# yang-song/score_sde_pytorch

Measured on AMD Instinct MI355X. Metric: pc_sampler_images_per_sec, higher is better.
Workload: dtype f32 via 3-way bf16 split, fp32 accumulate (the 1x1 / NIN / Linear GEMMs and the attention forward as exact-fp32 products on the BF16 matrix pipe, fp32 softmax; 3x3 convolutions and the attention backward on the fp32-MFMA kernels)

## Files before the change

### include/ssde.h

```cpp
#ifndef SSDE_H_
#define SSDE_H_

#include <stddef.h>
#include <stdint.h>

#ifdef __cplusplus
extern "C" {
#endif

#define SSDE_ABI_VERSION 10

enum {
  SSDE_PRO_NONE = 0,
  SSDE_PRO_GN = 1,
  SSDE_PRO_GN_SILU = 2,
  SSDE_PRO_SILU = 3
};

typedef struct ssde_src {
  const float* p0;
  const float* p1;
  int32_t c0, c1;
  int32_t pro_mode;
  int32_t gn_groups;
  const float* gn_mean;
  const float* gn_rstd;
  const float* gn_gamma;
  const float* gn_beta;
  uint32_t drop_thresh;
  float drop_scale;
  const uint32_t* drop_seed;
  uint32_t drop_salt;
  int32_t _pad;
} ssde_src;

typedef struct ssde_conv_args {
  ssde_src main;
  ssde_src aux;
  const float* w_main;
  const float* w_aux;
  int32_t n, h_in, w_in;
  int32_t h_out, w_out, c_out;
  int32_t ksize;
  int32_t stride;
  int32_t pad;
  int32_t tile;
  const float* bias;
  const float* chan_add;
  int32_t chan_add_ld;
  int32_t resid_post;
  const float* resid;
  float out_scale;
  uint32_t flags;
  float* dst;
  float* gn_part;
  float* wino_v;
  const float* gn_in_part0;
  const float* gn_in_part1;
  int32_t gn_in_slices0, gn_in_slices1;
  float gn_in_eps;
  int32_t _pad_gn_in;
} ssde_conv_args;

enum { SSDE_CONVF_V_GIVEN = 1u,
       SSDE_CONVF_BF16X6 = 2u,
       SSDE_CONVF_NO_KSPLIT = 4u,
       SSDE_CONVF_BKC8 = 8u,
       SSDE_CONVF_GEMM_PIPE = 16u,
       SSDE_CONVF_NO_GEMM_PIPE = 32u,
       SSDE_CONVF_X6_BM64 = 64u,
       SSDE_CONVF_X6_PF2 = 128u,
       SSDE_CONVF_NO_SMALL_COUT = 256u,
       SSDE_CONVF_X6_WIDE = 512u,
       SSDE_CONVF_X6_NO_WIDE = 1024u };
enum { SSDE_TILE_AUTO = 0, SSDE_TILE_256x64 = 1, SSDE_TILE_128x64 = 2, SSDE_TILE_64x64 = 3, SSDE_TILE_256x32 = 4,
       SSDE_TILE_WINOGRAD = 5,
       SSDE_TILE_WINOGRAD4 = 6,
       SSDE_TILE_WINOGRAD4R = 9 };

typedef struct ssde_gn_stats_args {
  const float* p0; const float* p1; int32_t c0, c1;
  int32_t n, hw, groups; float eps;
  float* mean; float* rstd;
  float* scratch;
  int32_t slices; int32_t _pad0;
} ssde_gn_stats_args;

typedef struct ssde_gn_finalize_args {
  const float* part0; const float* part1;
  int32_t c0, c1, slices0, slices1;
  int32_t n, groups; float eps; int32_t _pad0;
  float* mean; float* rstd;
} ssde_gn_finalize_args;

typedef struct ssde_upfirdn_args {
  ssde_src src;
  int32_t n, h_in, w_in, c;
  int32_t h_out, w_out;
  int32_t up, down, pad0, pad1;
  int32_t kh, kw;
  float k[16];
  float* dst;
  int32_t accumulate;
  int32_t _pad0;
  float* dst2;
} ssde_upfirdn_args;

typedef struct ssde_attn_args {
  const float* qkv; float* dst;
  int32_t n, l, c; float scale;
  uint32_t flags;
  int32_t _pad0;
} ssde_attn_args;
enum { SSDE_ATTNF_BF16X6 = 1u };

typedef struct ssde_embed_args {
  const float* cond;
  const float* w;
  float* dst;
  int32_t n, dim, kind, _pad0;
} ssde_embed_args;

typedef struct ssde_to_nhwc_args {
  const float* src; float* dst; int32_t n, c, h, w, c_pad; float a, b;
  int32_t mode;
  const float* v;
} ssde_to_nhwc_args;
typedef struct ssde_to_nchw_args {
  const float* src; float* dst; int32_t n, c, h, w, c_src;
  int32_t mode;
  const float* v;
  float alpha;
  int32_t accumulate;
} ssde_to_nchw_args;

typedef struct ssde_bias_act_args {
  const float* src; const float* bias; float* dst;
  int64_t numel; int32_t channels; int32_t inner;
  int32_t act;
  float alpha, scale;
  int32_t grad;
  const float* ref;
} ssde_bias_act_args;

typedef struct ssde_sumsq_args {
  const float* a; const float* b; float* out_a; float* out_b; int32_t n, per;
} ssde_sumsq_args;
typedef struct ssde_randn_args {
  float* dst; int64_t numel; uint64_t seed; const int32_t* step_ptr; int32_t stream_id; int32_t _pad0;
  const uint64_t* seed_ptr;
} ssde_randn_args;
typedef struct ssde_langevin_args {
  float* x; float* x_mean; const float* grad; const float* noise;
  const float* grad_sumsq; const float* noise_sumsq;
  const float* alpha_tab; const int32_t* step_ptr;
  int32_t n, per; float snr; int32_t _pad0;
} ssde_langevin_args;
// ... 313 lines not shown
```

### score_sde_pytorch_amd/_lib.py

```python
import ctypes as C
import os

_HERE = os.path.dirname(os.path.abspath(__file__))
LIB_PATH = os.environ.get("SSDE_LIB_PATH") or os.path.join(_HERE, "libssde_hip.so")
ABI_VERSION = 10

PRO_NONE, PRO_GN, PRO_GN_SILU, PRO_SILU = 0, 1, 2, 3
TILE_AUTO, TILE_256x64, TILE_128x64, TILE_64x64, TILE_256x32, TILE_WINOGRAD, TILE_WINOGRAD4 = 0, 1, 2, 3, 4, 5, 6
TILE_WINOGRAD4R = 9
TILES_WINOGRAD4 = (TILE_WINOGRAD4, TILE_WINOGRAD4R)
CONVF_V_GIVEN, CONVF_BF16X6, CONVF_NO_KSPLIT, CONVF_BKC8, CONVF_GEMM_PIPE, CONVF_NO_GEMM_PIPE, CONVF_X6_BM64, CONVF_X6_PF2, \
    CONVF_NO_SMALL_COUT, CONVF_X6_WIDE, CONVF_X6_NO_WIDE = 1, 2, 4, 8, 16, 32, 64, 128, 256, 512, 1024
WGRADF_DIRECT, WGRADF_F2, WGRADF_F4_FORCE, WGRADF_NO_STREAMK, WGRADF_NO_XCD_ORDER, WGRADF_1X1_CHUNKED, WGRADF_XVEC1 = 1, 2, 4, 8, 16, 32, 64
GNBWDF_THREE_KERNELS, GNBWDF_DEFER_PARAMS = 1, 2
(OP_CONV, OP_GN_STATS, OP_UPFIRDN, OP_ATTN, OP_EMBED, OP_TO_NHWC, OP_TO_NCHW, OP_BIAS_ACT, OP_SUMSQ,
 OP_RANDN, OP_LANGEVIN, OP_PREDICTOR, OP_FILL, OP_STEP_INC, OP_WGRAD, OP_COLSUM, OP_GN_BWD_REDUCE, OP_PROLOGUE_BWD,
 OP_ATTN_BWD, OP_PERTURB, OP_DSM_LOSS, OP_SUMSQ_FLAT, OP_ADAM, OP_MEMSET, OP_AXPY, OP_PACK, OP_PROJECT,
 OP_GN_FINALIZE, OP_PF_DRIFT, OP_HUTCH_DIV, OP_COLSUM_FINISH, OP_GN_BWD_FINISH) = range(1, 33)
FINISH_JOBS = 16
COLSUMF_DEFER = 1
PACK_CONV3, PACK_WINO3, PACK_MATRIX, PACK_VECTOR, PACK_WINO4, PACK_WINO4R = 1, 2, 3, 4, 5, 6

_fp = C.c_void_p


class Src(C.Structure):
    _fields_ = [("p0", _fp), ("p1", _fp), ("c0", C.c_int32), ("c1", C.c_int32),
                ("pro_mode", C.c_int32), ("gn_groups", C.c_int32),
                ("gn_mean", _fp), ("gn_rstd", _fp), ("gn_gamma", _fp), ("gn_beta", _fp),
                ("drop_thresh", C.c_uint32), ("drop_scale", C.c_float), ("drop_seed", _fp),
                ("drop_salt", C.c_uint32), ("_pad", C.c_int32)]


class ConvArgs(C.Structure):
    _fields_ = [("main", Src), ("aux", Src), ("w_main", _fp), ("w_aux", _fp),
                ("n", C.c_int32), ("h_in", C.c_int32), ("w_in", C.c_int32),
                ("h_out", C.c_int32), ("w_out", C.c_int32), ("c_out", C.c_int32),
                ("ksize", C.c_int32), ("stride", C.c_int32), ("pad", C.c_int32), ("tile", C.c_int32),
                ("bias", _fp), ("chan_add", _fp), ("chan_add_ld", C.c_int32), ("resid_post", C.c_int32),
                ("resid", _fp), ("out_scale", C.c_float), ("flags", C.c_uint32), ("dst", _fp), ("gn_part", _fp), ("wino_v", _fp),
                ("gn_in_part0", _fp), ("gn_in_part1", _fp), ("gn_in_slices0", C.c_int32), ("gn_in_slices1", C.c_int32),
                ("gn_in_eps", C.c_float), ("_pad_gn_in", C.c_int32)]


class GnStatsArgs(C.Structure):
    _fields_ = [("p0", _fp), ("p1", _fp), ("c0", C.c_int32), ("c1", C.c_int32),
                ("n", C.c_int32), ("hw", C.c_int32), ("groups", C.c_int32), ("eps", C.c_float),
                ("mean", _fp), ("rstd", _fp), ("scratch", _fp), ("slices", C.c_int32), ("_pad0", C.c_int32)]


class RkCombineArgs(C.Structure):
    _fields_ = [("y", _fp), ("k", _fp), ("n", C.c_int64), ("terms", C.c_int32), ("_pad0", C.c_int32), ("coef", C.c_double * 7),
                ("dst", _fp), ("dst32", _fp), ("n32", C.c_int64)]


class RkErrorArgs(C.Structure):
    _fields_ = [("y", _fp), ("y_new", _fp), ("k", _fp), ("n", C.c_int64), ("coef", C.c_double * 7), ("atol", C.c_double),
                ("rtol", C.c_double), ("partial", _fp), ("partial_len", C.c_int32), ("_pad0", C.c_int32), ("out", _fp)]


class PfDriftArgs(C.Structure):
    _fields_ = [("x", _fp), ("score", _fp), ("dst", _fp), ("numel", C.c_int64), ("a", C.c_float), ("g2", C.c_float), ("dyn", _fp)]


class OdeDyn(C.Structure):
    _fields_ = [("label", C.c_float), ("std", C.c_float), ("a", C.c_float), ("g2", C.c_float), ("dst", _fp)]


class HutchDivArgs(C.Structure):
    _fields_ = [("gx", _fp), ("eps", _fp), ("dst", _fp), ("dst_off", C.c_int64), ("n", C.c_int32), ("per", C.c_int32),
                ("a", C.c_float), ("g2", C.c_float), ("dyn", _fp)]


class GnFinalizeArgs(C.Structure):
    _fields_ = [("part0", _fp), ("part1", _fp), ("c0", C.c_int32), ("c1", C.c_int32), ("slices0", C.c_int32), ("slices1", C.c_int32),
                ("n", C.c_int32), ("groups", C.c_int32), ("eps", C.c_float), ("_pad0", C.c_int32), ("mean", _fp), ("rstd", _fp)]


class UpfirdnArgs(C.Structure):
    _fields_ = [("src", Src), ("n", C.c_int32), ("h_in", C.c_int32), ("w_in", C.c_int32), ("c", C.c_int32),
                ("h_out", C.c_int32), ("w_out", C.c_int32),
                ("up", C.c_int32), ("down", C.c_int32), ("pad0", C.c_int32), ("pad1", C.c_int32),
                ("kh", C.c_int32), ("kw", C.c_int32), ("k", C.c_float * 16), ("dst", _fp),
                ("accumulate", C.c_int32), ("_pad0", C.c_int32), ("dst2", _fp)]


class AttnArgs(C.Structure):
    _fields_ = [("qkv", _fp), ("dst", _fp), ("n", C.c_int32), ("l", C.c_int32), ("c", C.c_int32), ("scale", C.c_float),
                ("flags", C.c_uint32), ("_pad0", C.c_int32)]


class EmbedArgs(C.Structure):
    _fields_ = [("cond", _fp), ("w", _fp), ("dst", _fp), ("n", C.c_int32), ("dim", C.c_int32),
                ("kind", C.c_int32), ("_pad0", C.c_int32)]

# ... 120 lines not shown


class MemsetArgs(C.Structure):
    _fields_ = [("dst", _fp), ("bytes", C.c_int64), ("value", C.c_int32), ("_pad0", C.c_int32)]


class AxpyArgs(C.Structure):
    _fields_ = [("x", _fp), ("gate", _fp), ("dst", _fp), ("numel", C.c_int64), ("alpha", C.c_float), ("acc", C.c_int32)]


class PackDesc(C.Structure):
    _fields_ = [("src", _fp), ("src2", _fp), ("dst", _fp), ("kind", C.c_int32), ("cout", C.c_int32), ("cin", C.c_int32),
                ("cout_l", C.c_int32), ("cin_l", C.c_int32), ("flags", C.c_int32), ("r_off", C.c_int32), ("c_off", C.c_int32),
                ("n", C.c_int64)]


class PackArgs(C.Structure):
    _fields_ = [("table", _fp), ("count", C.c_int32), ("kind", C.c_int32), ("max_n", C.c_int64)]


class _OpUnion(C.Union):
    _fields_ = [("conv", ConvArgs), ("gn", GnStatsArgs), ("fir", UpfirdnArgs), ("attn", AttnArgs),
                ("embed", EmbedArgs), ("to_nhwc", ToNhwcArgs), ("to_nchw", ToNchwArgs), ("bias_act", BiasActArgs),
                ("sumsq", SumsqArgs), ("randn", RandnArgs), ("langevin", LangevinArgs), ("predictor", PredictorArgs),
                ("fill", FillArgs), ("step_inc", StepIncArgs),
                ("wgrad", WgradArgs), ("colsum", ColsumArgs), ("gn_bwd", GnBwdReduceArgs), ("pro_bwd", PrologueBwdArgs),
                ("attn_bwd", AttnBwdArgs), ("perturb", PerturbArgs), ("dsm_loss", DsmLossArgs),
                ("sumsq_flat", SumsqFlatArgs), ("adam", AdamArgs), ("memset", MemsetArgs), ("axpy", AxpyArgs),
                ("pack", PackArgs), ("project", ProjectArgs), ("gn_fin", GnFinalizeArgs),
                ("pf_drift", PfDriftArgs), ("hutch_div", HutchDivArgs), ("colsum_fin", ColsumFinishArgs), ("gn_bwd_fin", GnBwdFinishArgs)]


class Op(C.Structure):
    _fields_ = [("kind", C.c_int32), ("flops_class", C.c_int32), ("u", _OpUnion)]


_UNION_FIELD = {OP_CONV: "conv", OP_GN_STATS: "gn", OP_UPFIRDN: "fir", OP_ATTN: "attn", OP_EMBED: "embed",
                OP_TO_NHWC: "to_nhwc", OP_TO_NCHW: "to_nchw", OP_BIAS_ACT: "bias_act", OP_SUMSQ: "sumsq",
                OP_RANDN: "randn", OP_LANGEVIN: "langevin", OP_PREDICTOR: "predictor", OP_FILL: "fill",
                OP_STEP_INC: "step_inc", OP_WGRAD: "wgrad", OP_COLSUM: "colsum", OP_GN_BWD_REDUCE: "gn_bwd",
                OP_PROLOGUE_BWD: "pro_bwd", OP_ATTN_BWD: "attn_bwd", OP_PERTURB: "perturb", OP_DSM_LOSS: "dsm_loss",
                OP_SUMSQ_FLAT: "sumsq_flat", OP_ADAM: "adam", OP_MEMSET: "memset", OP_AXPY: "axpy", OP_PACK: "pack", OP_PROJECT: "project",
                OP_GN_FINALIZE: "gn_fin", OP_PF_DRIFT: "pf_drift", OP_HUTCH_DIV: "hutch_div", OP_COLSUM_FINISH: "colsum_fin",
                OP_GN_BWD_FINISH: "gn_bwd_fin"}

EXPORTS = ["ssde_conv2d", "ssde_groupnorm_stats", "ssde_upfirdn2d", "ssde_attention", "ssde_embed", "ssde_to_nhwc",
           "ssde_to_nchw", "ssde_fused_bias_act", "ssde_sumsq", "ssde_randn", "ssde_langevin_update",
           "ssde_predictor_update", "ssde_fill_from_table", "ssde_step_inc", "ssde_program_run",
           "ssde_program_run_timed", "ssde_graph_capture", "ssde_graph_launch", "ssde_graph_destroy",
           "ssde_abi_version", "ssde_sizeof_op", "ssde_last_error", "ssde_conv_lds_bytes",
           "ssde_conv_wgrad", "ssde_colsum", "ssde_gn_bwd_reduce", "ssde_prologue_bwd", "ssde_attention_bwd",
           "ssde_perturb", "ssde_dsm_loss", "ssde_sumsq_flat", "ssde_adam_clip_ema", "ssde_memset", "ssde_axpy",
           "ssde_wgrad_scratch_floats", "ssde_wgrad_wants_winograd4", "ssde_pack_weights", "ssde_project_update", "ssde_gn_finalize", "ssde_conv_gn_slices", "ssde_rk_combine", "ssde_rk_error_norm", "ssde_pf_drift", "ssde_hutch_div", "ssde_sample_update", "ssde_mfma_probe", "ssde_colsum_finish", "ssde_gn_bwd_finish", "ssde_gn_bwd_scratch_rows",
           "ssde_plan_load", "ssde_plan_load_file", "ssde_plan_destroy", "ssde_plan_info", "ssde_plan_param",
           "ssde_plan_refresh_weights", "ssde_unet_forward", "ssde_pc_reset", "ssde_pc_run", "ssde_pc_state",
           "ssde_train_step", "ssde_train_forward", "ssde_unet_backward", "ssde_plan_copy_io"]

_lib = None


def conv_route_flags(env=None):
    e = os.environ if env is None else env
    f = 0
    if e.get("SSDE_MATRIX", "").startswith("b"):
        f |= CONVF_BF16X6
    if e.get("SSDE_CONV_KSPLIT", "1") == "0":
        f |= CONVF_NO_KSPLIT
    if e.get("SSDE_CONV_BKC64", "") == "8":
        f |= CONVF_BKC8
    if e.get("SSDE_GEMM_PIPE", "") == "0":
        f |= CONVF_NO_GEMM_PIPE
    if e.get("SSDE_GEMM_PIPE", "") == "2":
        f |= CONVF_GEMM_PIPE
    if e.get("SSDE_X6_BM", "") == "64":
        f |= CONVF_X6_BM64
    if e.get("SSDE_X6_PF", "") == "2":
        f |= CONVF_X6_PF2
    if e.get("SSDE_CONV_SMALL", "1") == "0":
        f |= CONVF_NO_SMALL_COUT
    if e.get("SSDE_X6_WIDE", "") == "1":
        f |= CONVF_X6_WIDE
    if e.get("SSDE_X6_WIDE", "") == "0":
        f |= CONVF_X6_NO_WIDE
    return f


ATTNF_BF16X6 = 1


def attn_route_flags(env=None):
    e = os.environ if env is None else env
    return ATTNF_BF16X6 if e.get("SSDE_MATRIX", "").startswith("b") and e.get("SSDE_ATTN_X6", "1") != "0" else 0


def wgrad_route_flags(env=None):
    e = os.environ if env is None else env
    f = {"0": WGRADF_DIRECT, "2": WGRADF_F2, "44": WGRADF_F4_FORCE}.get(e.get("SSDE_WGRAD_WINOGRAD", ""), 0)
    if e.get("SSDE_WGRAD4_STREAMK", "1") == "0":
        f |= WGRADF_NO_STREAMK
    if e.get("SSDE_WGRAD4_XCD", "1") == "0":
        f |= WGRADF_NO_XCD_ORDER
    if e.get("SSDE_WGRAD_1X1_PIPELINED", "1") == "0":
        f |= WGRADF_1X1_CHUNKED
    if e.get("SSDE_WGRAD4_XVEC", "2") == "1":
        f |= WGRADF_XVEC1
    return f


def gn_bwd_route_flags(env=None):
    e = os.environ if env is None else env
    return GNBWDF_THREE_KERNELS if e.get("SSDE_GN_BWD_FUSED", "1") == "0" else 0


class SsdeError(RuntimeError):
    pass


def bind(lib):
    for name in EXPORTS:
        if not hasattr(lib, name):
            raise SsdeError("libssde_hip.so does not export %s" % name)
    lib.ssde_last_error.restype = C.c_char_p
    lib.ssde_program_run.argtypes = [C.POINTER(Op), C.c_int32, C.c_void_p]
    lib.ssde_program_run_timed.argtypes = [C.POINTER(Op), C.c_int32, C.c_void_p, C.POINTER(C.c_float)]
    lib.ssde_graph_capture.argtypes = [C.POINTER(Op), C.c_int32, C.c_void_p, C.POINTER(C.c_void_p)]
    lib.ssde_graph_launch.argtypes = [C.c_void_p, C.c_void_p]
    lib.ssde_graph_destroy.argtypes = [C.c_void_p]
    for name, typ in [("ssde_conv2d", ConvArgs), ("ssde_groupnorm_stats", GnStatsArgs), ("ssde_upfirdn2d", UpfirdnArgs),
                      ("ssde_attention", AttnArgs), ("ssde_embed", EmbedArgs), ("ssde_to_nhwc", ToNhwcArgs),
                      ("ssde_to_nchw", ToNchwArgs), ("ssde_fused_bias_act", BiasActArgs), ("ssde_sumsq", SumsqArgs),
                      ("ssde_randn", RandnArgs), ("ssde_langevin_update", LangevinArgs),
                      ("ssde_predictor_update", PredictorArgs), ("ssde_fill_from_table", FillArgs),
                      ("ssde_step_inc", StepIncArgs), ("ssde_conv_wgrad", WgradArgs), ("ssde_colsum", ColsumArgs),
                      ("ssde_gn_bwd_reduce", GnBwdReduceArgs), ("ssde_prologue_bwd", PrologueBwdArgs),
                      ("ssde_attention_bwd", AttnBwdArgs), ("ssde_perturb", PerturbArgs), ("ssde_dsm_loss", DsmLossArgs),
                      ("ssde_sumsq_flat", SumsqFlatArgs), ("ssde_adam_clip_ema", AdamArgs), ("ssde_memset", MemsetArgs),
                      ("ssde_axpy", AxpyArgs), ("ssde_pack_weights", PackArgs), ("ssde_project_update", ProjectArgs),
                      ("ssde_gn_finalize", GnFinalizeArgs), ("ssde_rk_combine", RkCombineArgs), ("ssde_hutch_div", HutchDivArgs), ("ssde_sample_update", SampleUpdateArgs),
                      ("ssde_rk_error_norm", RkErrorArgs), ("ssde_pf_drift", PfDriftArgs),
                      ("ssde_colsum_finish", ColsumFinishArgs), ("ssde_gn_bwd_finish", GnBwdFinishArgs)]:
        getattr(lib, name).argtypes = [C.POINTER(typ), C.c_void_p]
    lib.ssde_conv_lds_bytes.argtypes = [C.POINTER(ConvArgs)]
    lib.ssde_conv_gn_slices.argtypes = [C.POINTER(ConvArgs)]
    lib.ssde_wgrad_scratch_floats.argtypes = [C.POINTER(WgradArgs)]
    lib.ssde_wgrad_scratch_floats.restype = C.c_int64
    lib.ssde_wgrad_wants_winograd4.argtypes = [C.POINTER(WgradArgs)]
    lib.ssde_gn_bwd_scratch_rows.argtypes = [C.POINTER(GnBwdReduceArgs)]
    if lib.ssde_abi_version() != ABI_VERSION:
        raise SsdeError("ABI mismatch: library %d, binding %d" % (lib.ssde_abi_version(), ABI_VERSION))
    if lib.ssde_sizeof_op() != C.sizeof(Op):
        raise SsdeError("struct layout mismatch: sizeof(ssde_op) library %d, ctypes %d" % (lib.ssde_sizeof_op(), C.sizeof(Op)))
    return lib


def load():
    global _lib
    if _lib is not None:
        return _lib
    if not os.path.exists(LIB_PATH):
        raise SsdeError(
            "libssde_hip.so not found at %s -- build it with `python -c 'import __graft_entry__ as g; g.build()'` "
            "(score_sde_pytorch_amd has no CPU/eager fallback)" % LIB_PATH)
    lib = bind(C.CDLL(LIB_PATH))
    _lib = lib
    return lib

# ... 35 lines not shown
```

### score_sde_pytorch_amd/csrc/conv_mfma.hip

```cpp
#include "ssde_common.h"

typedef float f32x16 __attribute__((ext_vector_type(16)));

namespace {

struct ConvGeom {
  int N, Hin, Win, Hout, Wout, Cout, CoutPad;
  int stride, pad;
  int lTW, lTH;
  int tiles_x, tiles_per_img;
  int m_tiles, n_tiles;
};

struct ConvKParams {
  ssde_src main, aux;
  const float* w_main;
  const float* w_aux;
  ConvGeom g;
  const float* bias;
  const float* chan_add;
  int chan_add_ld;
  const float* resid;
  int resid_post;
  float scale;
// ... 107 lines not shown
        const int r = (q >> 1) / BN;
        const int tap = r % T, cb = r / T;
        const int cin8 = ch * NB8 + cb;
        if (cin8 < ncin8)
          bv[it] = *reinterpret_cast<const float4*>(
              wpk + ((size_t)(cin8 * T + tap) * g.CoutPad + n0 + j) * 8 + f * 4);
      }
    }
#pragma unroll
    for (int it = 0; it < MAXI; ++it) { mu[it] = 0.f; rs[it] = 1.f; }
    if (pro.gn && (c_base + f4 * 4) < Ctot) {
      gam = *reinterpret_cast<const float4*>(s.gn_gamma + c_base + f4 * 4);
      bet = *reinterpret_cast<const float4*>(s.gn_beta + c_base + f4 * 4);
      const int gidx = (c_base + f4 * 4) / cpg;
#pragma unroll
      for (int it = 0; it < MAXI; ++it)
        if (goff[it] >= 0) {
          mu[it] = s.gn_mean[gimg[it] * s.gn_groups + gidx];
          rs[it] = s.gn_rstd[gimg[it] * s.gn_groups + gidx];
        }
    }
  };
  auto store_stage = [&]() {
#pragma unroll
    for (int it = 0; it < MAXI; ++it) {
      if (goff[it] == -2) continue;
      float4 v = av[it];
      if (goff[it] >= 0 && chan_ok)
        v = ssde_pro_apply(v, mu[it], rs[it], gam, bet, (uint32_t)goff[it] * (uint32_t)Ctot + (uint32_t)(c_stage + f4 * 4), pro);
      const int q = tid + it * kThreads;
      *reinterpret_cast<float4*>(As + (q / F4) * LDA + f4 * 4) = v;
    }
#pragma unroll
    for (int it = 0; it < B_ITERS; ++it) {
      const int q = tid + it * kThreads;
      if (B_ITEMS % kThreads == 0 || q < B_ITEMS) {
        const int f = q & 1;
        const int j = (q >> 1) % BN;
        const int r = (q >> 1) / BN;
        const int tap = r % T, cb = r / T;
        *reinterpret_cast<float4*>(Bs + (tap * BN + j) * LDA + cb * 8 + f * 4) = bv[it];
      }
    }
  };

  if (ch0 >= ch1) return;
  load_stage(ch0);
  __syncthreads();
  store_stage();
  __syncthreads();
  for (int ch = ch0; ch < ch1; ++ch) {
    const bool has_next = ch + 1 < ch1;
    if (has_next) load_stage(ch + 1);
#pragma unroll
    for (int tap = 0; tap < T; ++tap) {
      const int dy = tap / KS, dx = tap % KS;
      const int aoff = (dy * HWd + dx) * LDA;
#pragma unroll
      for (int kk = 0; kk < NB8; ++kk) {
        float4 af[TM], bf[TN];
#pragma unroll
        for (int a = 0; a < TM; ++a) af[a] = *reinterpret_cast<const float4*>(As + hb[a] + aoff + kk * 8);
#pragma unroll
        for (int b = 0; b < TN; ++b) bf[b] = *reinterpret_cast<const float4*>(Bs + bb[b] + tap * BN * LDA + kk * 8);
#pragma unroll
        for (int a = 0; a < TM; ++a)
#pragma unroll
          for (int b = 0; b < TN; ++b) {
            acc[a][b] = __builtin_amdgcn_mfma_f32_32x32x2f32(af[a].x, bf[b].x, acc[a][b], 0, 0, 0);
            acc[a][b] = __builtin_amdgcn_mfma_f32_32x32x2f32(af[a].y, bf[b].y, acc[a][b], 0, 0, 0);
            acc[a][b] = __builtin_amdgcn_mfma_f32_32x32x2f32(af[a].z, bf[b].z, acc[a][b], 0, 0, 0);
            acc[a][b] = __builtin_amdgcn_mfma_f32_32x32x2f32(af[a].w, bf[b].w, acc[a][b], 0, 0, 0);
          }
      }
    }
    if (has_next) {
      __syncthreads();
      store_stage();
      __syncthreads();
    }
  }
}

template <int WM, int WN, int TM, int TN, bool HAS3, bool HAS1, int BKC3>
__global__ __launch_bounds__(kThreads, 2) void conv_mfma_kernel(const ConvKParams p) {
  constexpr int BM = WM * TM * 32, BN = WN * TN * 32;
  SSDE_LDS(smem);
  const ConvGeom& g = p.g;

  const int bid = blockIdx.x;
  const int xcd = bid & 7, l = bid >> 3;
  const int nt = l % g.n_tiles;
  const int ks = (l / g.n_tiles) % p.ksplit;
  const int mt = (l / (g.n_tiles * p.ksplit)) * 8 + xcd;
  if (mt >= g.m_tiles) return;

  const int IMGS = BM >> (g.lTW + g.lTH);
  const int img0 = (mt / g.tiles_per_img) * IMGS;
  const int trem = mt % g.tiles_per_img;
  const int ty = trem / g.tiles_x, tx = trem % g.tiles_x;
  const int n0 = nt * BN;

  const int wave = threadIdx.x >> 6;
  const int wm0 = (wave / WN) * (TM * 32);
  const int wn0 = (wave % WN) * (TN * 32);

  f32x16 acc[TM][TN];
#pragma unroll
  for (int a = 0; a < TM; ++a)
#pragma unroll
    for (int b = 0; b < TN; ++b)
#pragma unroll
      for (int r = 0; r < 16; ++r) acc[a][b][r] = 0.f;

  if constexpr (HAS3)
    conv_phase<3, BKC3, BM, BN, TM, TN, 5>(p.main, p.w_main, g, g.stride, g.pad, g.Hin, g.Win,
                                         img0, ty, tx, n0, wm0, wn0, acc, smem, ks, p.ksplit);
  if constexpr (HAS1)
    conv_phase<1, 32, BM, BN, TM, TN, (BM * 8) / kThreads>(p.aux, p.w_aux, g, 1, 0, g.Hout, g.Wout,
                                                          img0, ty, tx, n0, wm0, wn0, acc, smem, ks, p.ksplit);

  const int lane = threadIdx.x & 63;
  const int li = lane & 31, lh = lane >> 5;
  const int TW = 1 << g.lTW, TH = 1 << g.lTH;
  constexpr int LDT = BN + 4;
  __syncthreads();
#pragma unroll
  for (int b = 0; b < TN; ++b)
#pragma unroll
    for (int a = 0; a < TM; ++a)
#pragma unroll
      for (int r = 0; r < 16; ++r) {
        const int m = wm0 + a * 32 + (r & 3) + 8 * (r >> 2) + 4 * lh;
        smem[m * LDT + wn0 + b * 32 + li] = acc[a][b][r];
      }
  __syncthreads();
  auto pixfn = [&](int m, size_t& pix, int& img) {
    const int c = m & (TW - 1);
    const int rr = (m >> g.lTW) & (TH - 1);
    img = img0 + (m >> (g.lTW + g.lTH));
    const int oy = ty * TH + rr, ox = tx * TW + c;
    if (img >= g.N || oy >= g.Hout || ox >= g.Wout) return false;
    pix = ((size_t)img * g.Hout + oy) * g.Wout + ox;
    return true;
  };
  if constexpr (BM == 64 && BN == 64) if (p.ksplit == 2) {
    unsigned* sy = p.sync + 2 * (mt * g.n_tiles + nt);
    int* ticket = reinterpret_cast<int*>(smem + BM * LDT);
    if (threadIdx.x == 0) *ticket = (int)atomicAdd(sy, 1u);
    __syncthreads();
    const bool first = *ticket == 0;
    if (!first) {
      if (threadIdx.x == 0)
        while (__hip_atomic_load(sy + 1, __ATOMIC_RELAXED, __HIP_MEMORY_SCOPE_AGENT) == 0u) __builtin_amdgcn_s_sleep(4);
      __syncthreads();
    }
    constexpr int QN = BN / 4;
    constexpr int ITERS = BM * QN / kThreads;
    float* tp[ITERS];
    float* dp[ITERS];
    float o[ITERS][4];
#pragma unroll
    for (int it = 0; it < ITERS; ++it) {
      const int q = threadIdx.x + it * kThreads;
      const int m = q / QN, j = (q % QN) * 4;
      size_t pix; int img;
      const bool ok = pixfn(m, pix, img) && n0 + j < g.Cout;
      tp[it] = smem + m * LDT + j;
      dp[it] = ok ? p.dst + pix * g.Cout + n0 + j : nullptr;
    }
    if (first) {
#pragma unroll
      for (int it = 0; it < ITERS; ++it)
        if (dp[it]) {
#pragma unroll
          for (int k = 0; k < 4; ++k) __hip_atomic_store(dp[it] + k, tp[it][k], __ATOMIC_RELAXED, __HIP_MEMORY_SCOPE_AGENT);
        }
    } else {
#pragma unroll
      for (int it = 0; it < ITERS; ++it)
#pragma unroll
        for (int k = 0; k < 4; ++k)
          o[it][k] = dp[it] ? __hip_atomic_load(dp[it] + k, __ATOMIC_RELAXED, __HIP_MEMORY_SCOPE_AGENT) : 0.f;
#pragma unroll
      for (int it = 0; it < ITERS; ++it)
#pragma unroll
        for (int k = 0; k < 4; ++k) tp[it][k] += o[it][k];
    }
    if (first) {
      asm volatile("" ::: "memory");
      __builtin_amdgcn_s_waitcnt(0);
      __syncthreads();
      if (threadIdx.x == 0) atomicAdd(sy + 1, 1u);
      return;
    }
    __syncthreads();
    if (threadIdx.x == 0) { sy[0] = 0u; sy[1] = 0u; }
  }
  SsdeEpi e{p.bias, p.chan_add, p.chan_add_ld, p.resid, p.resid_post, p.scale, p.dst, g.Cout, p.gn_part};
  const int gn_entry = p.gn_part ? img0 * g.tiles_per_img + trem : -1;
  const int rpi_log2 = IMGS > 1 ? g.lTW + g.lTH : 30;
  ssde_store_tile<BM, BN, kThreads>(smem, LDT, n0, e, pixfn, gn_entry, rpi_log2, g.N * g.tiles_per_img);
}

struct TileCfg { int bm, bn; };
const TileCfg kTiles[5] = {{0, 0}, {256, 64}, {128, 64}, {64, 64}, {256, 32}};

struct ConvPlan {
  ConvKParams kp;
  int tile;
  int lds_bytes;
  int grid;
  bool has3, has1;
  int bkc;
  int gn_slices;
};

int src_check(const ssde_src& s, const char* what) {
  SSDE_REQUIRE(s.p0 != nullptr && s.c0 > 0, "conv: %s source missing", what);
  SSDE_REQUIRE(s.c0 % 4 == 0 && s.c1 % 4 == 0, "conv: %s channels must be multiples of 4 (got %d,%d)", what, s.c0, s.c1);
  SSDE_REQUIRE(s.c1 == 0 || s.p1 != nullptr, "conv: %s second tensor missing", what);
  SSDE_REQUIRE(s.c1 == 0 || s.c0 % 32 == 0, "conv: %s concat boundary must be a multiple of 32", what);
  if (s.pro_mode == SSDE_PRO_GN || s.pro_mode == SSDE_PRO_GN_SILU) {
    SSDE_REQUIRE(s.gn_groups > 0 && (s.c0 + s.c1) % s.gn_groups == 0 && ((s.c0 + s.c1) / s.gn_groups) % 4 == 0,
                 "conv: %s GroupNorm needs channels-per-group %% 4 == 0", what);
    SSDE_REQUIRE(s.gn_mean && s.gn_rstd && s.gn_gamma && s.gn_beta, "conv: %s GroupNorm pointers missing", what);
  }
  return SSDE_OK;
}

int pow2_floor(int v) { int p = 1; while (p * 2 <= v) p *= 2; return p; }

int halo_px(int bm, int w_out, int h_out, int stride, int ks, int* lTW, int* lTH) {
  int tw = pow2_floor(w_out < 16 ? w_out : 16);
  int th = bm / tw; if (th > h_out) th = h_out;
  th = pow2_floor(th);
  *lTW = ssde_ilog2(tw); *lTH = ssde_ilog2(th);
  const int imgs = bm / (tw * th);
  return imgs * ((th - 1) * stride + ks) * ((tw - 1) * stride + ks);
}

int make_plan(const ssde_conv_args* a, ConvPlan* pl) {
  SSDE_REQUIRE(a && a->dst, "conv: null args");
  pl->has3 = a->ksize != 0;
  pl->has1 = a->aux.p0 != nullptr;
  SSDE_REQUIRE(pl->has3 || pl->has1, "conv: neither a k x k nor a 1 x 1 source");
  SSDE_REQUIRE(a->ksize == 0 || a->ksize == 3, "conv: ksize must be 0 or 3 (1x1 goes through aux)");
  SSDE_REQUIRE(a->n > 0 && a->h_out > 0 && a->w_out > 0 && a->c_out > 0, "conv: bad output shape");
  if (pl->has3) {
    if (int rc = src_check(a->main, "main")) return rc;
    SSDE_REQUIRE(a->w_main, "conv: w_main missing");
    SSDE_REQUIRE(a->stride == 1 || a->stride == 2, "conv: stride must be 1 or 2");
    SSDE_REQUIRE((a->h_in + 2 * a->pad - 3) / a->stride + 1 >= a->h_out && (a->w_in + 2 * a->pad - 3) / a->stride + 1 >= a->w_out,
                 "conv: output %dx%d larger than input %dx%d stride %d pad %d allows", a->h_out, a->w_out, a->h_in, a->w_in, a->stride, a->pad);
  }
  if (pl->has1) {
    if (int rc = src_check(a->aux, "aux")) return rc;
    SSDE_REQUIRE(a->w_aux, "conv: w_aux missing");
  }
  const int M = a->n * a->h_out * a->w_out;
  int tile = a->tile;
  if (tile == SSDE_TILE_AUTO) {
    if (a->c_out <= 32) tile = SSDE_TILE_256x32;
    else {
      const int nt = ssde_cdiv(a->c_out, 64);
      if (ssde_cdiv(M, 256) * nt >= 512) tile = SSDE_TILE_256x64;
      else if (ssde_cdiv(M, 128) * nt >= 384) tile = SSDE_TILE_128x64;
      else tile = SSDE_TILE_64x64;
    }
    if (a->w_out * a->h_out * a->n < kTiles[tile].bm && tile != SSDE_TILE_256x32) tile = SSDE_TILE_64x64;
  }
  SSDE_REQUIRE(tile >= 1 && tile <= 4, "conv: bad tile id %d", tile);
  (void)SSDE_TILE_WINOGRAD4;
  (void)SSDE_TILE_WINOGRAD;
  int lTW = 0, lTH = 0;
  pl->bkc = 8;
  const bool deep_ok = !(a->flags & SSDE_CONVF_BKC8);
  if (pl->has3) {
    while (true) {
      const int px = halo_px(kTiles[tile].bm, a->w_out, a->h_out, a->stride, 3, &lTW, &lTH);
      pl->bkc = (deep_ok && tile == SSDE_TILE_64x64 && px * (SSDE_CONV_BKC64 / 4) <= 5 * kThreads) ? SSDE_CONV_BKC64 : 8;
      if (px * 2 <= 5 * kThreads) break;
      SSDE_REQUIRE(tile != SSDE_TILE_64x64, "conv: halo too large for any tile");
      tile = (tile == SSDE_TILE_256x32) ? SSDE_TILE_64x64 : tile + 1;
    }
  } else {
    halo_px(kTiles[tile].bm, a->w_out, a->h_out, 1, 1, &lTW, &lTH);
  }
  const int bm = kTiles[tile].bm, bn = kTiles[tile].bn;
  const int tw = 1 << lTW, th = 1 << lTH, imgs = bm / (tw * th);

  ConvKParams& kp = pl->kp;
  kp.main = a->main; kp.aux = a->aux; kp.w_main = a->w_main; kp.w_aux = a->w_aux;
  ConvGeom& g = kp.g;
  g.N = a->n; g.Hin = a->h_in; g.Win = a->w_in; g.Hout = a->h_out; g.Wout = a->w_out;
  g.Cout = a->c_out; g.CoutPad = ssde_cdiv(a->c_out, 64) * 64;
  g.stride = pl->has3 ? a->stride : 1; g.pad = pl->has3 ? a->pad : 0;
  g.lTW = lTW; g.lTH = lTH;
  g.tiles_x = ssde_cdiv(a->w_out, tw);
  g.tiles_per_img = g.tiles_x * ssde_cdiv(a->h_out, th);
  g.m_tiles = ssde_cdiv(a->n, imgs) * g.tiles_per_img;
  g.n_tiles = ssde_cdiv(a->c_out, bn);
  kp.bias = a->bias; kp.chan_add = a->chan_add; kp.chan_add_ld = a->chan_add_ld;
  kp.resid = a->resid; kp.resid_post = a->resid_post; kp.scale = a->out_scale; kp.dst = a->dst;
  kp.gn_part = a->gn_part;
  const bool gn_ok = a->c_out % 4 == 0 && (imgs == 1 || (g.tiles_per_img == 1 && tw * th >= kThreads / (bn / 4)));
  pl->gn_slices = gn_ok ? g.tiles_per_img * (kThreads / 64) : 0;
  SSDE_REQUIRE(!a->gn_part || pl->gn_slices > 0, "conv: GroupNorm partials need one image per tile and c_out %% 4 == 0");

  int lds = 0;
  if (pl->has3) {
    const int px = imgs * ((th - 1) * g.stride + 3) * ((tw - 1) * g.stride + 3);
    const int lda = pl->bkc + 4;
    lds = (((px * lda + 3) & ~3) + 9 * bn * lda) * 4;
  }
  if (pl->has1) {
    const int l1 = (bm * 36 + bn * 36) * 4;
    if (l1 > lds) lds = l1;
  }
  const int epi_bytes = bm * (bn + 4) * 4 + 16;
  pl->lds_bytes = lds > epi_bytes ? lds : epi_bytes;
  pl->tile = tile;
  const bool split_ok = !(a->flags & SSDE_CONVF_NO_KSPLIT);
  const int wgs = ssde_cdiv(g.m_tiles, 8) * 8 * g.n_tiles;
  const int ctot = pl->has3 ? a->main.c0 + a->main.c1 : 0;
  kp.ksplit = (split_ok && pl->has3 && tile == SSDE_TILE_64x64 && wgs <= 320 && ctot >= 128 && a->c_out % 4 == 0 &&
               a->resid != a->dst && g.m_tiles * g.n_tiles <= kSyncSlots / 4) ? 2 : 1;
  kp.sync = nullptr;
  pl->grid = wgs * kp.ksplit;
  return SSDE_OK;
}

template <int WM, int WN, int TM, int TN, int BKC3 = 8>
int launch_cfg(ConvPlan& pl, hipStream_t st) {
  dim3 grid(pl.grid), block(kThreads);
  if (pl.kp.ksplit == 2) {
    pl.kp.sync = ssde_conv_sync_slots(pl.kp.g.m_tiles * pl.kp.g.n_tiles);
    SSDE_REQUIRE(pl.kp.sync, "conv: no hand-over slots for a split reduction");
  }
#define SSDE_CONV_LAUNCH(H3, H1)                                                                     \
  do {                                                                                               \
    auto kfn = conv_mfma_kernel<WM, WN, TM, TN, H3, H1, BKC3>;                                       \
    static std::atomic<bool> attr_set{false};             \
    if (!attr_set) {                                                                                 \
      SSDE_HIP_CHECK(hipFuncSetAttribute(reinterpret_cast<const void*>(kfn),                         \
                                         hipFuncAttributeMaxDynamicSharedMemorySize, 160 * 1024));   \
      attr_set = true;                                                                               \
    }                                                                                                \
    hipLaunchKernelGGL(kfn, grid, block, pl.lds_bytes, st, pl.kp);                                   \
  } while (0)
  if (pl.has3 && pl.has1) SSDE_CONV_LAUNCH(true, true);
  else if (pl.has3) SSDE_CONV_LAUNCH(true, false);
  else SSDE_CONV_LAUNCH(false, true);
#undef SSDE_CONV_LAUNCH
  SSDE_LAUNCH_CHECK();
  return SSDE_OK;
}

}

unsigned* ssde_conv_sync_slots(int need) {
  static std::atomic<unsigned> cursor{0};
  if (need <= 0 || need > kSyncSlots / 4) return nullptr;
  unsigned cur = cursor.load(std::memory_order_relaxed), at, next;
  do {
    at = cur % (unsigned)kSyncSlots;
    if (at + (unsigned)need > (unsigned)kSyncSlots) at = 0;
    next = at + (unsigned)need;
  } while (!cursor.compare_exchange_weak(cur, next, std::memory_order_relaxed));
  unsigned* base = nullptr;
  if (hipGetSymbolAddress(reinterpret_cast<void**>(&base), HIP_SYMBOL(g_conv_sync)) != hipSuccess) return nullptr;
  return base + 2 * (size_t)at;
}

typedef int (*ssde_wino_launcher)(const ssde_conv_args*, void*, int*);
static ssde_wino_launcher wino_launcher(int tile) {
  switch (tile) {
    case SSDE_TILE_WINOGRAD: return ssde_conv_wino_launch;
    case SSDE_TILE_WINOGRAD4: return ssde_conv_wino4_launch;
    case SSDE_TILE_WINOGRAD4R: return ssde_conv_wino4r_launch;
    default: return nullptr;
  }
}

extern "C" int ssde_conv2d(const ssde_conv_args* a, void* stream) {
  if (a && a->gn_in_part0 && !ssde_wino4_xform_merges_gn(a)) {
    const ssde_src& s = a->main;
    SSDE_REQUIRE(s.gn_mean && s.gn_rstd && s.gn_groups > 0 && a->ksize != 0, "conv: gn_in_part0 needs a k x k main source with a GroupNorm prologue");
    ssde_gn_finalize_args f;
    f.part0 = a->gn_in_part0; f.part1 = s.c1 > 0 ? a->gn_in_part1 : nullptr;
    f.c0 = s.c0; f.c1 = s.c1; f.slices0 = a->gn_in_slices0; f.slices1 = s.c1 > 0 ? a->gn_in_slices1 : 0;
    f.n = a->n; f.groups = s.gn_groups; f.eps = a->gn_in_eps;
    f.mean = const_cast<float*>(s.gn_mean); f.rstd = const_cast<float*>(s.gn_rstd);
    if (int rc = ssde_gn_finalize(&f, stream)) return rc;
  }
  if (a) {
    if (ssde_wino_launcher fn = wino_launcher(a->tile)) {
      if (a->tile == SSDE_TILE_WINOGRAD4R && !(a->flags & SSDE_CONVF_V_GIVEN)) {
        int lds = 0;
        if (int rc = fn(a, nullptr, &lds)) return rc;
        if (int rc = ssde_wino4_xform_vq_launch(a, stream)) return rc;
      }
      return fn(a, stream, nullptr);
    }
  }
  if (a && a->dst && ssde_conv1x1_wants(a)) return ssde_conv1x1_launch(a, stream, nullptr);
  if (a && a->dst && ssde_conv_small_wants(a)) return ssde_conv_small_launch(a, stream, nullptr);
  ConvPlan pl;
  if (int rc = make_plan(a, &pl)) return rc;
  hipStream_t st = static_cast<hipStream_t>(stream);
  switch (pl.tile) {
    case SSDE_TILE_256x64: return launch_cfg<4, 1, 2, 2>(pl, st);
    case SSDE_TILE_128x64: return launch_cfg<4, 1, 1, 2>(pl, st);
    case SSDE_TILE_64x64:  return pl.bkc == 8 ? launch_cfg<2, 2, 1, 1>(pl, st) : launch_cfg<2, 2, 1, 1, SSDE_CONV_BKC64>(pl, st);
    case SSDE_TILE_256x32: return launch_cfg<4, 1, 2, 1>(pl, st);
  }
  ssde_set_error("conv: unreachable tile %d", pl.tile);
  return SSDE_EINVAL;
}

extern "C" int ssde_conv_gn_slices(const ssde_conv_args* a) {
  if (!a || a->c_out % 4 != 0) return 0;
  ssde_conv_args q = *a;
  q.gn_part = nullptr;
  if (ssde_wino_launcher fn = wino_launcher(q.tile)) {
    int s = 0;
    if (fn(&q, reinterpret_cast<void*>(1), &s)) return 0;
    return s;
  }
  if (q.dst && ssde_conv1x1_wants(&q)) {
    const int hw = q.h_out * q.w_out;
    if (hw % 64 == 0) return (hw / 64) * 4;
    return (hw >= 8 && hw < 64 && 64 % hw == 0) ? 4 : 0;
  }
  if (q.dst && ssde_conv_small_wants(&q)) return 0;
  ConvPlan pl;
  if (make_plan(&q, &pl)) return 0;
  return pl.gn_slices;
}

extern "C" int ssde_conv_lds_bytes(const ssde_conv_args* a) {
  if (ssde_wino_launcher fn = a ? wino_launcher(a->tile) : nullptr) {
    int lds = 0;
    if (int rc = fn(a, nullptr, &lds)) return rc;
    return lds;
  }
  if (a && a->dst && ssde_conv1x1_wants(a)) {
    int lds = 0;
    if (int rc = ssde_conv1x1_launch(a, nullptr, &lds)) return rc;
    return lds;
  }
  if (a && a->dst && ssde_conv_small_wants(a)) {
    int lds = 0;
    if (int rc = ssde_conv_small_launch(a, nullptr, &lds)) return rc;
    return lds;
  }
  ConvPlan pl;
  if (int rc = make_plan(a, &pl)) return rc;
  return pl.lds_bytes;
}
```

Before: 5.480.

## Add bf16x6 direct 3x3 convolution path for the 64x64 MFMA tile

Adds a direct-convolution phase that splits activations and weights into three bf16 planes in LDS. It accumulates with the bf16 matrix instructions (bf16x6 emulation of fp32) instead of fp32 MFMA, for the 64x64 tile when the BF16X6 flag is set and the halo fits. The aim is higher matrix throughput on convolutions that go through the generic MFMA kernel. In exchange it adds split overhead, triple-plane LDS use and a new kernel variant. An environment switch can turn it off.

```diff
diff --git a/include/ssde.h b/include/ssde.h
--- a/include/ssde.h
+++ b/include/ssde.h
@@ -72,7 +72,8 @@
        SSDE_CONVF_X6_PF2 = 128u,
        SSDE_CONVF_NO_SMALL_COUT = 256u,
        SSDE_CONVF_X6_WIDE = 512u,
-       SSDE_CONVF_X6_NO_WIDE = 1024u };
+       SSDE_CONVF_X6_NO_WIDE = 1024u,
+       SSDE_CONVF_X6_NO_DIRECT = 2048u };
 enum { SSDE_TILE_AUTO = 0, SSDE_TILE_256x64 = 1, SSDE_TILE_128x64 = 2, SSDE_TILE_64x64 = 3, SSDE_TILE_256x32 = 4,
        SSDE_TILE_WINOGRAD = 5,
        SSDE_TILE_WINOGRAD4 = 6,
diff --git a/score_sde_pytorch_amd/_lib.py b/score_sde_pytorch_amd/_lib.py
--- a/score_sde_pytorch_amd/_lib.py
+++ b/score_sde_pytorch_amd/_lib.py
@@ -10,7 +10,7 @@
 TILE_WINOGRAD4R = 9
 TILES_WINOGRAD4 = (TILE_WINOGRAD4, TILE_WINOGRAD4R)
 CONVF_V_GIVEN, CONVF_BF16X6, CONVF_NO_KSPLIT, CONVF_BKC8, CONVF_GEMM_PIPE, CONVF_NO_GEMM_PIPE, CONVF_X6_BM64, CONVF_X6_PF2, \
-    CONVF_NO_SMALL_COUT, CONVF_X6_WIDE, CONVF_X6_NO_WIDE = 1, 2, 4, 8, 16, 32, 64, 128, 256, 512, 1024
+    CONVF_NO_SMALL_COUT, CONVF_X6_WIDE, CONVF_X6_NO_WIDE, CONVF_X6_NO_DIRECT = 1, 2, 4, 8, 16, 32, 64, 128, 256, 512, 1024, 2048
 WGRADF_DIRECT, WGRADF_F2, WGRADF_F4_FORCE, WGRADF_NO_STREAMK, WGRADF_NO_XCD_ORDER, WGRADF_1X1_CHUNKED, WGRADF_XVEC1 = 1, 2, 4, 8, 16, 32, 64
 GNBWDF_THREE_KERNELS, GNBWDF_DEFER_PARAMS = 1, 2
 (OP_CONV, OP_GN_STATS, OP_UPFIRDN, OP_ATTN, OP_EMBED, OP_TO_NHWC, OP_TO_NCHW, OP_BIAS_ACT, OP_SUMSQ,
@@ -297,6 +297,8 @@
         f |= CONVF_X6_WIDE
     if e.get("SSDE_X6_WIDE", "") == "0":
         f |= CONVF_X6_NO_WIDE
+    if e.get("SSDE_X6_DIRECT", "1") == "0":
+        f |= CONVF_X6_NO_DIRECT
     return f
 
 
diff --git a/score_sde_pytorch_amd/csrc/conv_mfma.hip b/score_sde_pytorch_amd/csrc/conv_mfma.hip
--- a/score_sde_pytorch_amd/csrc/conv_mfma.hip
+++ b/score_sde_pytorch_amd/csrc/conv_mfma.hip
@@ -213,7 +213,183 @@
   }
 }
 
-template <int WM, int WN, int TM, int TN, bool HAS3, bool HAS1, int BKC3>
+constexpr int kX6HaloItems = 5;
+template <int KS, int MAXI>
+__device__ __forceinline__ void conv_phase_x6(const ssde_src& s, const float* __restrict__ wpk,
+                                              const ConvGeom& g, int stride, int pad, int Hs, int Ws,
+                                              int img0, int ty, int tx, int n0, int wm0, int wn0,
+                                              f32x16& acc, float* smem, int ks, int ksplit) {
+  constexpr int T = KS * KS;
+  constexpr int BKC = 16, F4 = BKC / 4, BM = 64, BN = 64;
+  constexpr int PIX = BKC * 2;
+  const int tid = threadIdx.x;
+  const int lane = tid & 63;
+  const int li = lane & 31, lh = lane >> 5;
+  const int TW = 1 << g.lTW, TH = 1 << g.lTH;
+  const int IMGS = BM >> (g.lTW + g.lTH);
+  const int HWd = (TW - 1) * stride + KS;
+  const int HH = (TH - 1) * stride + KS;
+  const int halo_px = IMGS * HH * HWd;
+  const int items = halo_px * F4;
+  const int planeA = halo_px * PIX;
+  constexpr int planeB = T * BN * PIX;
+  char* As = reinterpret_cast<char*>(smem);
+  char* Bs = As + 3 * planeA;
+
+  const int f4 = tid % F4;
+  int goff[MAXI];
+  int gimg[MAXI];
+#pragma unroll
+  for (int it = 0; it < MAXI; ++it) {
+    const int q = tid + it * kThreads;
+    goff[it] = -2;
+    gimg[it] = 0;
+    if (q < items) {
+      const int hp = q / F4;
+      const int il = hp / (HH * HWd);
+      const int rem = hp - il * (HH * HWd);
+      const int hy = rem / HWd;
+      const int hx = rem - hy * HWd;
+      const int iy = ty * TH * stride - pad + hy;
+      const int ix = tx * TW * stride - pad + hx;
+      const int img = img0 + il;
+      const bool inb = (img < g.N) && (iy >= 0) && (iy < Hs) && (ix >= 0) && (ix < Ws);
+      goff[it] = inb ? (img * Hs + iy) * Ws + ix : -1;
+      gimg[it] = img;
+    }
+  }
+  int hb;
+  {
+    const int m = wm0 + li;
+    const int c = m & (TW - 1);
+    const int r = (m >> g.lTW) & (TH - 1);
+    const int il = m >> (g.lTW + g.lTH);
+    hb = ((il * HH + r * stride) * HWd + c * stride) * PIX + lh * 16;
+  }
+  const int bb = (wn0 + li) * PIX + lh * 16;
+
+  const int Ctot = s.c0 + s.c1;
+  const int ncin8 = (Ctot + 7) >> 3;
+  const int nchunks = (Ctot + BKC - 1) / BKC;
+  const int ch0 = nchunks * ks / ksplit, ch1 = nchunks * (ks + 1) / ksplit;
+  const SsdePro pro = ssde_pro_decode(s);
+  const int cpg = pro.gn ? Ctot / s.gn_groups : 1;
+  constexpr int B_ITEMS = T * BN * F4;
+  constexpr int B_ITERS = (B_ITEMS + kThreads - 1) / kThreads;
+
+  float4 av[MAXI];
+  float4 bv[B_ITERS];
+  float mu[MAXI], rs[MAXI];
+  float4 gam = make_float4(1.f, 1.f, 1.f, 1.f), bet = make_float4(0.f, 0.f, 0.f, 0.f);
+  bool chan_ok = false;
+  int c_stage = 0;
+
+  auto load_stage = [&](int ch) {
+    const int c_base = ch * BKC;
+    c_stage = c_base;
+    const float* base;
+    int C, cc;
+    if (c_base < s.c0) { base = s.p0; C = s.c0; cc = c_base; }
+    else               { base = s.p1; C = s.c1; cc = c_base - s.c0; }
+    const int cthr = cc + f4 * 4;
+    chan_ok = cthr < C;
+#pragma unroll
+    for (int it = 0; it < MAXI; ++it) {
+      av[it] = make_float4(0.f, 0.f, 0.f, 0.f);
+      if (goff[it] >= 0 && chan_ok)
+        av[it] = *reinterpret_cast<const float4*>(base + (size_t)goff[it] * C + cthr);
+    }
+#pragma unroll
+    for (int it = 0; it < B_ITERS; ++it) {
+      const int q = tid + it * kThreads;
+      bv[it] = make_float4(0.f, 0.f, 0.f, 0.f);
+      if (B_ITEMS % kThreads == 0 || q < B_ITEMS) {
+        const int f = q & 1;
+        const int j = (q >> 1) % BN;
+        const int r = (q >> 1) / BN;
+        const int tap = r % T, cb = r / T;
+        const int cin8 = ch * 2 + cb;
+        if (cin8 < ncin8)
+          bv[it] = *reinterpret_cast<const float4*>(
+              wpk + ((size_t)(cin8 * T + tap) * g.CoutPad + n0 + j) * 8 + f * 4);
+      }
+    }
+#pragma unroll
+    for (int it = 0; it < MAXI; ++it) { mu[it] = 0.f; rs[it] = 1.f; }
+    if (pro.gn && (c_base + f4 * 4) < Ctot) {
+      gam = *reinterpret_cast<const float4*>(s.gn_gamma + c_base + f4 * 4);
+      bet = *reinterpret_cast<const float4*>(s.gn_beta + c_base + f4 * 4);
+      const int gidx = (c_base + f4 * 4) / cpg;
+#pragma unroll
+      for (int it = 0; it < MAXI; ++it)
+        if (goff[it] >= 0) {
+          mu[it] = s.gn_mean[gimg[it] * s.gn_groups + gidx];
+          rs[it] = s.gn_rstd[gimg[it] * s.gn_groups + gidx];
+        }
+    }
+  };
+  auto store_stage = [&]() {
+    uint2 q0, q1, q2;
+#pragma unroll
+    for (int it = 0; it < MAXI; ++it) {
+      if (goff[it] == -2) continue;
+      float4 v = av[it];
+      if (goff[it] >= 0 && chan_ok)
+        v = ssde_pro_apply(v, mu[it], rs[it], gam, bet, (uint32_t)goff[it] * (uint32_t)Ctot + (uint32_t)(c_stage + f4 * 4), pro);
+      const int q = tid + it * kThreads;
+      char* d = As + (q / F4) * PIX + f4 * 8;
+      ssde_split3(v, q0, q1, q2);
+      *reinterpret_cast<uint2*>(d) = q0;
+      *reinterpret_cast<uint2*>(d + planeA) = q1;
+      *reinterpret_cast<uint2*>(d + 2 * planeA) = q2;
+    }
+#pragma unroll
+    for (int it = 0; it < B_ITERS; ++it) {
+      const int q = tid + it * kThreads;
+      if (B_ITEMS % kThreads == 0 || q < B_ITEMS) {
+        const int f = q & 1;
+        const int j = (q >> 1) % BN;
+        const int r = (q >> 1) / BN;
+        const int tap = r % T, cb = r / T;
+        char* d = Bs + (tap * BN + j) * PIX + (cb * 8 + f * 4) * 2;
+        ssde_split3(bv[it], q0, q1, q2);
+        *reinterpret_cast<uint2*>(d) = q0;
+        *reinterpret_cast<uint2*>(d + planeB) = q1;
+        *reinterpret_cast<uint2*>(d + 2 * planeB) = q2;
+      }
+    }
+  };
+
+  if (ch0 >= ch1) return;
+  load_stage(ch0);
+  __syncthreads();
+  store_stage();
+  __syncthreads();
+  for (int ch = ch0; ch < ch1; ++ch) {
+    const bool has_next = ch + 1 < ch1;
+    if (has_next) load_stage(ch + 1);
+#pragma unroll
+    for (int tap = 0; tap < T; ++tap) {
+      const int dy = tap / KS, dx = tap % KS;
+      const char* ap = As + hb + (dy * HWd + dx) * PIX;
+      const char* bp = Bs + bb + tap * BN * PIX;
+      ssde_u32x4 A[3], B[3];
+#pragma unroll
+      for (int q = 0; q < 3; ++q) {
+        A[q] = *reinterpret_cast<const ssde_u32x4*>(ap + q * planeA);
+        B[q] = *reinterpret_cast<const ssde_u32x4*>(bp + q * planeB);
+      }
+      SSDE_MFMA_BF16X6(acc, A, B);
+    }
+    if (has_next) {
+      __syncthreads();
+      store_stage();
+      __syncthreads();
+    }
+  }
+}
+
+template <int WM, int WN, int TM, int TN, bool HAS3, bool HAS1, int BKC3, bool X6 = false>
 __global__ __launch_bounds__(kThreads, 2) void conv_mfma_kernel(const ConvKParams p) {
   constexpr int BM = WM * TM * 32, BN = WN * TN * 32;
   SSDE_LDS(smem);
@@ -244,12 +420,21 @@
 #pragma unroll
       for (int r = 0; r < 16; ++r) acc[a][b][r] = 0.f;
 
-  if constexpr (HAS3)
-    conv_phase<3, BKC3, BM, BN, TM, TN, 5>(p.main, p.w_main, g, g.stride, g.pad, g.Hin, g.Win,
-                                         img0, ty, tx, n0, wm0, wn0, acc, smem, ks, p.ksplit);
-  if constexpr (HAS1)
-    conv_phase<1, 32, BM, BN, TM, TN, (BM * 8) / kThreads>(p.aux, p.w_aux, g, 1, 0, g.Hout, g.Wout,
-                                                          img0, ty, tx, n0, wm0, wn0, acc, smem, ks, p.ksplit);
+  if constexpr (X6) {
+    static_assert(BM == 64 && BN == 64 && TM == 1 && TN == 1, "bf16x6 direct convolution: the 64 x 64 tile only");
+    if constexpr (HAS3)
+      conv_phase_x6<3, kX6HaloItems>(p.main, p.w_main, g, g.stride, g.pad, g.Hin, g.Win,
+                                     img0, ty, tx, n0, wm0, wn0, acc[0][0], smem, ks, p.ksplit);
+    if constexpr (HAS1)
+      conv_phase_x6<1, 1>(p.aux, p.w_aux, g, 1, 0, g.Hout, g.Wout, img0, ty, tx, n0, wm0, wn0, acc[0][0], smem, ks, p.ksplit);
+  } else {
+    if constexpr (HAS3)
+      conv_phase<3, BKC3, BM, BN, TM, TN, 5>(p.main, p.w_main, g, g.stride, g.pad, g.Hin, g.Win,
+                                           img0, ty, tx, n0, wm0, wn0, acc, smem, ks, p.ksplit);
+    if constexpr (HAS1)
+      conv_phase<1, 32, BM, BN, TM, TN, (BM * 8) / kThreads>(p.aux, p.w_aux, g, 1, 0, g.Hout, g.Wout,
+                                                            img0, ty, tx, n0, wm0, wn0, acc, smem, ks, p.ksplit);
+  }
 
   const int lane = threadIdx.x & 63;
   const int li = lane & 31, lh = lane >> 5;
@@ -344,6 +529,7 @@
   int grid;
   bool has3, has1;
   int bkc;
+  bool x6;
   int gn_slices;
 };
 
@@ -420,6 +606,9 @@
   }
   const int bm = kTiles[tile].bm, bn = kTiles[tile].bn;
   const int tw = 1 << lTW, th = 1 << lTH, imgs = bm / (tw * th);
+  pl->x6 = (a->flags & SSDE_CONVF_BF16X6) && !(a->flags & SSDE_CONVF_X6_NO_DIRECT) && tile == SSDE_TILE_64x64 &&
+           (!pl->has3 || imgs * ((th - 1) * a->stride + 3) * ((tw - 1) * a->stride + 3) * 4 <= kX6HaloItems * kThreads);
+  if (pl->x6) pl->bkc = 16;
 
   ConvKParams& kp = pl->kp;
   kp.main = a->main; kp.aux = a->aux; kp.w_main = a->w_main; kp.w_aux = a->w_aux;
@@ -440,14 +629,19 @@
   SSDE_REQUIRE(!a->gn_part || pl->gn_slices > 0, "conv: GroupNorm partials need one image per tile and c_out %% 4 == 0");
 
   int lds = 0;
-  if (pl->has3) {
-    const int px = imgs * ((th - 1) * g.stride + 3) * ((tw - 1) * g.stride + 3);
-    const int lda = pl->bkc + 4;
-    lds = (((px * lda + 3) & ~3) + 9 * bn * lda) * 4;
-  }
-  if (pl->has1) {
-    const int l1 = (bm * 36 + bn * 36) * 4;
-    if (l1 > lds) lds = l1;
+  if (pl->x6) {
+    if (pl->has3) lds = 3 * 32 * (imgs * ((th - 1) * g.stride + 3) * ((tw - 1) * g.stride + 3) + 9 * bn);
+    if (pl->has1 && 3 * 32 * (bm + bn) > lds) lds = 3 * 32 * (bm + bn);
+  } else {
+    if (pl->has3) {
+      const int px = imgs * ((th - 1) * g.stride + 3) * ((tw - 1) * g.stride + 3);
+      const int lda = pl->bkc + 4;
+      lds = (((px * lda + 3) & ~3) + 9 * bn * lda) * 4;
+    }
+    if (pl->has1) {
+      const int l1 = (bm * 36 + bn * 36) * 4;
+      if (l1 > lds) lds = l1;
+    }
   }
   const int epi_bytes = bm * (bn + 4) * 4 + 16;
   pl->lds_bytes = lds > epi_bytes ? lds : epi_bytes;
@@ -462,7 +656,7 @@
   return SSDE_OK;
 }
 
-template <int WM, int WN, int TM, int TN, int BKC3 = 8>
+template <int WM, int WN, int TM, int TN, int BKC3 = 8, bool X6 = false>
 int launch_cfg(ConvPlan& pl, hipStream_t st) {
   dim3 grid(pl.grid), block(kThreads);
   if (pl.kp.ksplit == 2) {
@@ -471,7 +665,7 @@
   }
 #define SSDE_CONV_LAUNCH(H3, H1)                                                                     \
   do {                                                                                               \
-    auto kfn = conv_mfma_kernel<WM, WN, TM, TN, H3, H1, BKC3>;                                       \
+    auto kfn = conv_mfma_kernel<WM, WN, TM, TN, H3, H1, BKC3, X6>;                                       \
     static std::atomic<bool> attr_set{false};             \
     if (!attr_set) {                                                                                 \
       SSDE_HIP_CHECK(hipFuncSetAttribute(reinterpret_cast<const void*>(kfn),                         \
@@ -543,7 +737,9 @@
   switch (pl.tile) {
     case SSDE_TILE_256x64: return launch_cfg<4, 1, 2, 2>(pl, st);
     case SSDE_TILE_128x64: return launch_cfg<4, 1, 1, 2>(pl, st);
-    case SSDE_TILE_64x64:  return pl.bkc == 8 ? launch_cfg<2, 2, 1, 1>(pl, st) : launch_cfg<2, 2, 1, 1, SSDE_CONV_BKC64>(pl, st);
+    case SSDE_TILE_64x64:
+      if (pl.x6) return launch_cfg<2, 2, 1, 1, 16, true>(pl, st);
+      return pl.bkc == 8 ? launch_cfg<2, 2, 1, 1>(pl, st) : launch_cfg<2, 2, 1, 1, SSDE_CONV_BKC64>(pl, st);
     case SSDE_TILE_256x32: return launch_cfg<4, 1, 2, 1>(pl, st);
   }
   ssde_set_error("conv: unreachable tile %d", pl.tile);
```

Result: faster. 5.557, median of 6 (+1.4%).
